# Dimitrinov74/Domain-Specific-Image-Compression

Hardware: AMD Instinct MI355X
Metric: 256x256 satellite patches encoded/s per GPU; bpp + MS-SSIM vs reference (higher is better)
Workload: dtype f32 (Winograd contractions as split-bf16 MFMA with fp32 accumulate); 1 GPU; batch=64/GPU 256x256x3 synthetic patches, modelv2 encode->decode (g_a,h_a,round,h_s,Student-t/Gaussian rate,g_s) + bpp + MS-SSIM[.3,.5,.2] on GPU + CDF tables and range coder (z,y strings) on GPU [BASELINE config 3]; global_batch=64, parallelism=per-image sharding x1, one all-reduce of 4 fp64, weights=synthetic seed 1 (checkpoints absent from the reference)

## Files before the change

### domain-specific-image-compression_amd/csrc/dsic_math.h

```cpp
#pragma once
#include <stdint.h>

#if defined(__HIPCC__)
#define DM_HD __host__ __device__ inline
#else
#define DM_HD inline
#endif

namespace dsic {
namespace dm {

#define DM_LN2_HI 6.93147180369123816490e-01
#define DM_LN2_LO 1.90821492927058770002e-10
#define DM_INV_LN2 1.44269504088896338700e+00
#define DM_SQRT2 1.41421356237309514547e+00
#define DM_INV_SQRT_PI 5.64189583547756279280e-01
#define DM_HALF_LOG_2PI 9.18938533204672780563e-01

DM_HD double from_bits(uint64_t b) {
  union {
    uint64_t u;
    double d;
  } v;
  v.u = b;
// ... 120 lines not shown
  for (int m = 1; m <= 400; ++m) {
    const double dm_ = (double)m, m2 = 2.0 * dm_;
    double aa = dm_ * (b - dm_) * x / ((qam + m2) * (a + m2));
    d = 1.0 + aa * d;
    if (d < TINY && d > -TINY) d = TINY;
    c = 1.0 + aa / c;
    if (c < TINY && c > -TINY) c = TINY;
    d = 1.0 / d;
    h = h * d * c;
    aa = -(a + dm_) * (qab + dm_) * x / ((a + m2) * (qap + m2));
    d = 1.0 + aa * d;
    if (d < TINY && d > -TINY) d = TINY;
    c = 1.0 + aa / c;
    if (c < TINY && c > -TINY) c = TINY;
    d = 1.0 / d;
    const double del = d * c;
    h = h * del;
    double dev = del - 1.0;
    if (dev < 0) dev = -dev;
    if (dev < 3e-16) break;
  }
  return h;
}

DM_HD double betainc(double a, double b, double x, double xc) {
  if (x <= 0.0) return 0.0;
  if (xc <= 0.0) return 1.0;
  const double lbeta = lgamma(a + b) - lgamma(a) - lgamma(b);
  const double front = exp(lbeta + a * log(x) + b * log(xc));
  if (x < (a + 1.0) / (a + b + 2.0)) return front * betacf(a, b, x) / a;
  return 1.0 - front * betacf(b, a, xc) / b;
}

DM_HD double student_t_cdf(double t, double nu) {
  const double t2 = t * t;
  const double den = nu + t2;
  const double x = nu / den, xc = t2 / den;
  const double tail = 0.5 * betainc(0.5 * nu, 0.5, x, xc);
  return t > 0 ? 1.0 - tail : tail;
}


DM_HD double erf_pos(double u) {
  if (u < 1.5) {
    const double u2 = u * u;
    double term = u, sum = u;
    for (int n = 1; n < 200; ++n) {
      term = term * (2.0 * u2) / (double)(2 * n + 1);
      sum = sum + term;
      if (term < sum * 1e-17) break;
    }
    return 2.0 * DM_INV_SQRT_PI * exp(-u2) * sum;
  }
  if (u > 6.0) return 1.0;
  return 1.0 - erfc_pos(u);
}

DM_HD float erff_rn(float a) {
  const double u = (double)a;
  if (u != u) return a;
  return u < 0 ? -(float)erf_pos(-u) : (float)erf_pos(u);
}

DM_HD float gaussian_cdf_f32(float x) {
  const float a = x / 1.41421354f;
  const float e = erff_rn(a);
  const float s = 1.0f + e;
  return 0.5f * s;
}

DM_HD float sum_f32_torch(const float* p, int n) {
// ... 57 lines not shown
```

### domain-specific-image-compression_amd/csrc/entropy.hip

```cpp
#include "common.h"
#include "dsic_math.h"

namespace dsic {

__global__ __launch_bounds__(256) void support_kernel(const float* __restrict__ y,
                                                      const float* __restrict__ z,
                                                      int* __restrict__ meta, int64_t ny, int64_t nz,
                                                      int tail) {
  __shared__ float red[2][4];
  __shared__ int bad_any;
  const int b = blockIdx.x;
  for (int which = 0; which < 2; ++which) {
    const float* p = which ? z + (size_t)b * nz : y + (size_t)b * ny;
    const int64_t n = which ? nz : ny;
    float mn = p[0], mx = p[0];
    bool bad = false;
    for (int64_t i = threadIdx.x; i < n; i += 256) {
      const float v = p[i];
      bad |= !(fabsf(v) < 1.0e9f);
      mn = fminf(mn, v);
      mx = fmaxf(mx, v);
    }
#pragma unroll
    for (int o = 32; o > 0; o >>= 1) {
      mn = fminf(mn, __shfl_down(mn, o, 64));
      mx = fmaxf(mx, __shfl_down(mx, o, 64));
    }
    if (threadIdx.x == 0) bad_any = 0;
    __syncthreads();
    if ((threadIdx.x & 63) == 0) {
      red[0][threadIdx.x >> 6] = mn;
      red[1][threadIdx.x >> 6] = mx;
    }
    if (__any(bad) && (threadIdx.x & 63) == 0) atomicOr(&bad_any, 1);
// ... 42 lines not shown
  __builtin_amdgcn_wave_barrier();
  for (int k = lane; k < L; k += 64) {
    uint32_t u16 = 0;
    if (k > 0) {
      float sc = F[k - 1] * 65535.0f;
      if (sc < 0.0f) sc = 0.0f;
      if (sc > 65535.0f) sc = 65535.0f;
      u16 = (uint32_t)sc;
    }
    out[k] = (uint16_t)((u16 * (uint32_t)(65536 - L)) / 65535u + (uint32_t)k);
  }
}

template <bool STUDENT>
__global__ __launch_bounds__(256) void tables_kernel(const float* __restrict__ sigma,
                                                     const float* __restrict__ nu, int sb,
                                                     const int* __restrict__ meta, int meta_off,
                                                     uint16_t* __restrict__ tables, int C, int Lmax,
                                                     int ntables, int* __restrict__ err) {
  extern __shared__ float shm[];
  const int wave = threadIdx.x >> 6, lane = threadIdx.x & 63;
  const int tid = blockIdx.x * 4 + wave;
  if (tid >= ntables) return;
  const int b = tid / C, c = tid % C;
  const int smin = meta[4 * b + meta_off], L = meta[4 * b + meta_off + 1];
  if (L > Lmax || L < 1) {
    if (lane == 0) atomicOr(err, 1);
    return;
  }
  float* F = shm + (size_t)wave * (2 * Lmax + 1);
  float* pmf = F + Lmax + 1;
  const float sg = sigma[(size_t)b * sb + c];
  const float nv = STUDENT ? nu[(size_t)b * sb + c] : 0.0f;
  for (int k = lane; k <= L; k += 64)
    F[k] = STUDENT ? dm::table_cdf_student(smin, k, sg, nv) : dm::table_cdf_gauss(smin, k, sg);
  __builtin_amdgcn_s_waitcnt(0xc07f);
  __builtin_amdgcn_wave_barrier();
  finish_table_wave(F, L, tables + ((size_t)b * C + c) * Lmax, pmf, lane);
}

__device__ __forceinline__ void put_bits(uint32_t* out32, int64_t cap_bits, int64_t off, uint32_t v,
                                         int len, int* overflow) {
  if (off + len > cap_bits) {
    *overflow = 1;
    return;
  }
  const int64_t w = off >> 5;
  const int s = (int)(off & 31), space = 32 - s;
  if (len <= space) {
    atomicOr(out32 + w, __builtin_bswap32(v << (space - len)));
  } else {
    const int rest = len - space;
    atomicOr(out32 + w, __builtin_bswap32(v >> rest));
    atomicOr(out32 + w + 1, __builtin_bswap32(v << (32 - rest)));
  }
}

__device__ __forceinline__ void put_ones(uint32_t* out32, int64_t cap_bits, int64_t off, uint32_t count,
                                         int* overflow) {
  while (count > 0) {
    const int len = count > 32 ? 32 : (int)count;
    put_bits(out32, cap_bits, off, len == 32 ? 0xFFFFFFFFu : ((1u << len) - 1u), len, overflow);
    off += len;
    count -= len;
  }
}

#ifndef ENC_SELECT
#define ENC_SELECT 1
#endif
template <int J>
__device__ __forceinline__ void wlane(uint32_t& rec, uint32_t v) {
  asm volatile("v_writelane_b32 %0, %1, %2" : "+v"(rec) : "s"(v), "n"(J));
}

template <int J>
__device__ __forceinline__ uint32_t rlane(uint32_t v) {
  uint32_t r;
  asm volatile("v_readlane_b32 %0, %1, %2" : "=s"(r) : "v"(v), "n"(J));
  return r;
}

template <int J>
__device__ __forceinline__ void enc_step(uint32_t& low, uint32_t& lowm1, uint32_t& span, uint32_t& cl,
                                         uint32_t& ch, uint32_t clo16, uint32_t chi16, uint32_t& rec_low,
                                         uint32_t& rec_high) {
  const uint32_t cl_next = J < 63 ? rlane<(J < 63 ? J + 1 : 63)>(clo16) : 0u;
  const uint32_t ch_next = J < 63 ? rlane<(J < 63 ? J + 1 : 63)>(chi16) : 0u;
  uint32_t lo_add, hi_add;
#if ENC_SELECT
  {
    const uint32_t ml = __umulhi(span, cl), mh = __umulhi(span, ch);
    lo_add = span ? ml : cl;
    hi_add = span ? mh : ch;
  }
// ... 168 lines not shown
        if (pendv == 0) {
          put_bits(dst32, cap_bits, off, bitsv, (int)nbv, &overflow);
        } else {
          const uint32_t first = bitsv >> (nbv - 1);
          put_bits(dst32, cap_bits, off, first, 1, &overflow);
          if (!first) put_ones(dst32, cap_bits, off + 1, pendv, &overflow);
          else if (off + 1 + (int64_t)pendv > cap_bits) overflow = 1;
          if (nbv > 1)
            put_bits(dst32, cap_bits, off + 1 + pendv, bitsv & ((1u << (nbv - 1)) - 1u), (int)nbv - 1, &overflow);
        }
      }
      base_bits += (int64_t)__builtin_amdgcn_readlane((int)incl, 63);
    }
    cur = nxt;
    sym1 = sym2;
  }
  pending += 1;
  const uint32_t bit = low < 0x40000000u ? 0u : 1u;
  if (lane == 0) {
    put_bits(dst32, cap_bits, base_bits, bit, 1, &overflow);
    if (!bit) put_ones(dst32, cap_bits, base_bits + 1, pending, &overflow);
    else if (base_bits + 1 + (int64_t)pending > cap_bits) overflow = 1;
  }
  const int64_t total_bits = base_bits + 1 + (int64_t)pending;
  if (__any(overflow)) {
    if (lane == 0) atomicOr(err, 4);
  }
  if (lane == 0) lengths[2 * b + which] = (int)((total_bits + 7) >> 3);
}

struct SplitGeom {
  int B, M, HWy, N, HWz, Lmax, per_element_y;
  int64_t ny, nz;
  __device__ __forceinline__ void stream(int s, int& which, int& b, int64_t& n, int64_t& base) const {
    which = s < B ? 1 : 0;
    b = which ? s : s - B;
    n = which ? ny : nz;
    base = which ? (int64_t)b * ny : (int64_t)B * ny + (int64_t)b * nz;
  }
};

__global__ __launch_bounds__(256) void enc_pack_kernel(const float* __restrict__ y, const float* __restrict__ z,
                                                       const int* __restrict__ meta, const uint16_t* __restrict__ tab_y,
                                                       const uint16_t* __restrict__ tab_z, SplitGeom G,
                                                       uint32_t* __restrict__ pairs, int* __restrict__ err) {
  int which, b;
  int64_t n, base;
  G.stream(blockIdx.y, which, b, n, base);
  const int HW = which ? G.HWy : G.HWz, Lmax = G.Lmax;
  const bool per_element = which && G.per_element_y;
  const float* sym = which ? y + (size_t)b * n : z + (size_t)b * n;
  const uint16_t* tab = (which ? tab_y + (size_t)b * (per_element ? (size_t)G.M * G.HWy : (size_t)G.M) * Lmax
                               : tab_z + (size_t)b * G.N * Lmax);
  const int smin = meta[4 * b + (which ? 0 : 2)], L = meta[4 * b + (which ? 1 : 3)];
  if (L > Lmax || L < 1) return;
  for (int64_t g = (int64_t)blockIdx.x * 256 + threadIdx.x; g < n; g += (int64_t)gridDim.x * 256) {
    const int c = (int)(g / HW);
    int sc = (int)sym[g] - smin;
    if (sc < 0 || sc >= L) {
      atomicOr(err, 2);
      sc = 0;
    }
    const uint16_t* t = tab + (size_t)(per_element ? g : (int64_t)c) * Lmax;
    const uint32_t c_low = t[sc];
    const uint32_t c_high = (sc == L - 1) ? 0x10000u : (uint32_t)t[sc + 1];
    pairs[base + g] = c_low | ((c_high - 1u) << 16);
  }
}

template <int J>
__device__ __forceinline__ void chain_step(uint32_t& low, uint32_t& lowm1, uint32_t& span, uint32_t& cl, uint32_t& ch,
                                           uint32_t pv, uint32_t& rec_low, uint32_t& rec_high) {
  const uint32_t pn = J < 63 ? rlane<(J < 63 ? J + 1 : 63)>(pv) : 0u;
// ... 61 lines not shown
    chain_steps8<40>(low, lowm1, span, cl, ch, cur, rl, rh);
    chain_steps8<48>(low, lowm1, span, cl, ch, cur, rl, rh);
    chain_steps8<56>(low, lowm1, span, cl, ch, cur, rl, rh);
    __builtin_amdgcn_raw_buffer_store_b32(rl, rlo, voff, g * 4u, 0);
    __builtin_amdgcn_raw_buffer_store_b32(rh, rhi, voff, g * 4u, 0);
    cur = n1;
    n1 = n2;
  }
  const int cnt = (int)((uint32_t)n - g);
  if (cnt > 0) {
    uint32_t rl = 0, rh = 0;
    for (int j = 0; j < cnt; ++j) {
      const uint32_t pr = __builtin_amdgcn_readlane(cur, j);
      const uint32_t cl = pr << 16, ch = (pr & 0xFFFF0000u) + 0x10000u;
      const uint32_t lo_add = span ? __umulhi(span, cl) : cl;
      const uint32_t hi_add = ch ? (span ? __umulhi(span, ch) : ch) : span;
      const uint32_t low1 = low + lo_add, high1 = lowm1 + hi_add, span1 = hi_add - lo_add;
      asm volatile("s_mov_b32 m0, %4\n\ts_nop 3\n\tv_writelane_b32 %0, %2, m0\n\tv_writelane_b32 %1, %3, m0"
                   : "+v"(rl), "+v"(rh)
                   : "s"(low1), "s"(high1), "s"(j));
      const int nb = __builtin_clz(low1 ^ high1);
      const int m = __builtin_clz(((high1 | ~low1) << 1) << nb);
      const int sh = nb + m;
      span = span1 << sh;
      low = (low1 << sh) & 0x7FFFFFFFu;
      lowm1 = low - 1u;
    }
    __builtin_amdgcn_raw_buffer_store_b32(rl, rlo, voff, g * 4u, 0);
    __builtin_amdgcn_raw_buffer_store_b32(rh, rhi, voff, g * 4u, 0);
  }
  if (threadIdx.x == 0) final_low[s] = low;
}

constexpr int PLACE_THREADS = 1024;

__global__ __launch_bounds__(PLACE_THREADS) void enc_place_kernel(const int* __restrict__ meta, SplitGeom G,
                                                                  const uint32_t* __restrict__ rec_low,
                                                                  const uint32_t* __restrict__ rec_high,
                                                                  const uint32_t* __restrict__ final_low,
                                                                  uint8_t* __restrict__ out, int64_t cap_y,
                                                                  int64_t cap_z, int* __restrict__ lengths,
                                                                  int* __restrict__ err) {
  __shared__ uint32_t sc_a[PLACE_THREADS], sc_t[PLACE_THREADS];
  __shared__ uint64_t sc_l[PLACE_THREADS];
  const int s = blockIdx.x, tid = threadIdx.x;
  int which, b;
  int64_t n, base;
  G.stream(s, which, b, n, base);
  const int L = meta[4 * b + (which ? 1 : 3)];
  if (L > G.Lmax || L < 1) {
    if (tid == 0) {
      atomicOr(err, 1);
      lengths[2 * b + which] = 0;
    }
    return;
  }
  const int64_t stride = cap_z + cap_y;
  uint32_t* dst32 = (uint32_t*)(out + (size_t)b * stride + (which ? cap_z : 0));
  const int64_t cap_bits = (which ? cap_y : cap_z) * 8;
  const uint32_t* rlo = rec_low + base;
  const uint32_t* rhi = rec_high + base;
  const int64_t per = (n + PLACE_THREADS - 1) / PLACE_THREADS;
  const int64_t j0 = (int64_t)tid * per < n ? (int64_t)tid * per : n;
  const int64_t j1 = j0 + per < n ? j0 + per : n;

  uint32_t t = 0, head = 0;
  uint64_t len = 0;
  for (int64_t j = j0; j < j1; ++j) {
    const uint32_t lo = rlo[j], hi = rhi[j];
    const uint32_t nb = (uint32_t)__builtin_clz(lo ^ hi);
    const uint32_t m = (uint32_t)__builtin_clz((((hi | ~lo) << nb) << 1) | 1u);
    if (nb) {
      len += nb + t;
      head = 1;
      t = 0;
    }
    t += m;
  }
  sc_a[tid] = head ? 0u : 1u;
  sc_t[tid] = t;
  __syncthreads();
  for (int o = 1; o < PLACE_THREADS; o <<= 1) {
    uint32_t pa = 1, pt = 0;
    if (tid >= o) {
      pa = sc_a[tid - o];
      pt = sc_t[tid - o];
    }
    __syncthreads();
    if (tid >= o) {
      const uint32_t a = sc_a[tid];
      sc_t[tid] = (a ? pt : 0u) + sc_t[tid];
      sc_a[tid] = pa & a;
    }
    __syncthreads();
  }
  const uint32_t carry_in = tid ? sc_t[tid - 1] : 0u;
  const uint32_t pend_final = sc_t[PLACE_THREADS - 1];
  const uint64_t mylen = len + (head ? (uint64_t)carry_in : 0u);
  __syncthreads();
  sc_l[tid] = mylen;
  __syncthreads();
  for (int o = 1; o < PLACE_THREADS; o <<= 1) {
    const uint64_t v = tid >= o ? sc_l[tid - o] : 0u;
    __syncthreads();
    sc_l[tid] += v;
    __syncthreads();
  }
  const int64_t total = (int64_t)sc_l[PLACE_THREADS - 1];
  int64_t off = (int64_t)(sc_l[tid] - mylen);

  int overflow = 0;
  uint32_t pend = carry_in;
  for (int64_t j = j0; j < j1; ++j) {
    const uint32_t lo = rlo[j], hi = rhi[j];
    const uint32_t nbv = (uint32_t)__builtin_clz(lo ^ hi);
    const uint32_t m = (uint32_t)__builtin_clz((((hi | ~lo) << nbv) << 1) | 1u);
    if (nbv) {
      const uint32_t bitsv = lo >> (32u - nbv);
      const uint32_t pendv = pend;
      if (pendv == 0) {
        put_bits(dst32, cap_bits, off, bitsv, (int)nbv, &overflow);
      } else {
        const uint32_t first = bitsv >> (nbv - 1);
        put_bits(dst32, cap_bits, off, first, 1, &overflow);
        if (!first) put_ones(dst32, cap_bits, off + 1, pendv, &overflow);
        else if (off + 1 + (int64_t)pendv > cap_bits) overflow = 1;
        if (nbv > 1)
          put_bits(dst32, cap_bits, off + 1 + pendv, bitsv & ((1u << (nbv - 1)) - 1u), (int)nbv - 1, &overflow);
      }
      off += nbv + pendv;
      pend = 0;
    }
    pend += m;
  }
  if (tid == 0) {
    const uint32_t pending = pend_final + 1u;
    const uint32_t bit = final_low[s] < 0x40000000u ? 0u : 1u;
    put_bits(dst32, cap_bits, total, bit, 1, &overflow);
    if (!bit) put_ones(dst32, cap_bits, total + 1, pending, &overflow);
    else if (total + 1 + (int64_t)pending > cap_bits) overflow = 1;
    lengths[2 * b + which] = (int)((total + 1 + (int64_t)pending + 7) >> 3);
  }
  if (overflow) atomicOr(err, 4);
}

__global__ __launch_bounds__(256) void range_decode_kernel(const uint8_t* __restrict__ in,
                                                           int64_t stride,
                                                           const int* __restrict__ lengths, int lstride,
                                                           int loff, const int* __restrict__ meta,
                                                           int meta_off,
                                                           const uint16_t* __restrict__ tables, int Lmax,
                                                           int C, int HW, float* __restrict__ out,
                                                           int* __restrict__ err, int B,
                                                           int per_element) {
  const int lane = threadIdx.x & 63;
  const int b = __builtin_amdgcn_readfirstlane(blockIdx.x * (blockDim.x >> 6) + (threadIdx.x >> 6));
  if (b >= B) return;
  const int smin = meta[4 * b + meta_off], L = meta[4 * b + meta_off + 1];
  if (L > Lmax || L < 1) {
    if (lane == 0) atomicOr(err, 1);
    return;
  }
  const uint16_t* gt = tables + (size_t)b * (per_element ? (size_t)C * HW : (size_t)C) * Lmax;
  const uint32_t* src32 = (const uint32_t*)(in + (size_t)b * stride);
  const int nbytes = lengths[b * lstride + loff];
  const int ndw = (nbytes + 3) >> 2;
  const int64_t n = (int64_t)C * HW;
  float* dst = out + (size_t)b * n;

  auto load_window = [&](int w0) -> uint32_t {
    const int k = w0 + lane;
    uint32_t v = 0;
    if (k < ndw) {
      v = __builtin_bswap32(src32[k]);
      const int valid = nbytes - 4 * k;
      if (valid < 4) v &= 0xFFFFFFFFu << (8 * (4 - valid));
// ... 131 lines not shown
          c_high = 0x10000u;
        }
      }
      ck0 = ck0_next;
      if (new_row) {
        row += 1;
        in_row = 0;
      } else {
        in_row += 1;
      }
      const int sidx = cnt - 1;
      if (lane == 0) dst[g] = (float)(sidx + smin);
      const uint32_t hi_add = (uint32_t)(((uint64_t)r * c_high + c_high) >> 16);
      const uint32_t lo_add = (uint32_t)(((uint64_t)r * c_low + c_low) >> 16);
      high = (low - 1u) + hi_add;
      low = low + lo_add;
      const int nb = __builtin_clz(low ^ high);
      low <<= nb;
      high = (high << nb) | ((1u << nb) - 1u);
      value = nb ? ((value << nb) | take(nb)) : value;
      const uint32_t e3 = (low << 1) & ~(high << 1);
      const int m = __builtin_clz(~e3);
      low = (low << m) & 0x7FFFFFFFu;
      high = (high << m) | 0x80000000u | ((1u << m) - 1u);
      value = m ? (((value << m) | take(m)) ^ 0x80000000u) : value;
    }
  }
}

}

using namespace dsic;

extern "C" int dsic_latent_support(const float* y_nchw, const float* z_nchw, int* meta, int B,
                                   int64_t n_y, int64_t n_z, int tail, void* stream) {
  DSIC_REQUIRE(y_nchw && z_nchw && meta, "latent_support: null pointer");
  DSIC_REQUIRE(B > 0 && n_y > 0 && n_z > 0 && tail >= 0, "latent_support: bad argument");
  hipLaunchKernelGGL(support_kernel, dim3(B), dim3(256), 0, (hipStream_t)stream, y_nchw, z_nchw, meta,
                     n_y, n_z, tail);
  return check_launch("latent_support");
}

static int tables_launch(bool student, const float* sigma, const float* nu, int per_image,
                         const int* meta, int meta_off, uint16_t* tables, int B, int C, int Lmax,
                         int* err, hipStream_t st) {
  DSIC_REQUIRE(sigma && meta && tables && err && (!student || nu), "cdf_tables: null pointer");
  DSIC_REQUIRE(B > 0 && C > 0 && Lmax >= 1 && Lmax <= 1000, "cdf_tables: Lmax=%d must be in [1,1000]", Lmax);
  const int ntables = B * C;
  const size_t shm = (size_t)4 * (2 * Lmax + 1) * sizeof(float);
  const int sb = per_image ? C : 0;
  if (student)
    hipLaunchKernelGGL(tables_kernel<true>, dim3(ceil_div(ntables, 4)), dim3(256), shm, st, sigma, nu, sb,
                       meta, meta_off, tables, C, Lmax, ntables, err);
  else
    hipLaunchKernelGGL(tables_kernel<false>, dim3(ceil_div(ntables, 4)), dim3(256), shm, st, sigma, nu, sb,
                       meta, meta_off, tables, C, Lmax, ntables, err);
  return check_launch("cdf_tables");
}

extern "C" int dsic_cdf_tables_gauss(const float* sigma_z, const int* meta, uint16_t* tables, int B,
                                     int N, int Lmax, int* err, void* stream) {
  return tables_launch(false, sigma_z, nullptr, 0, meta, 2, tables, B, N, Lmax, err, (hipStream_t)stream);
}

extern "C" int dsic_cdf_tables_student(const float* sigma, const float* nu, const int* meta,
                                       uint16_t* tables, int B, int rows, int Lmax, int* err,
                                       void* stream) {
  return tables_launch(true, sigma, nu, 1, meta, 0, tables, B, rows, Lmax, err, (hipStream_t)stream);
}

extern "C" int dsic_range_encode(const float* y_nchw, const float* z_nchw, const int* meta,
                                 const uint16_t* tab_y, const uint16_t* tab_z, int Lmax, int B, int M,
                                 int HWy, int N, int HWz, uint8_t* out, int64_t cap_y, int64_t cap_z,
                                 int* lengths, int* err, int streams_per_wg, int per_element_y,
                                 void* stream) {
  DSIC_REQUIRE(y_nchw && z_nchw && meta && tab_y && tab_z && out && lengths && err,
               "range_encode: null pointer");
  DSIC_REQUIRE(B > 0 && M > 0 && N > 0 && HWy > 0 && HWz > 0, "range_encode: empty latent");
  DSIC_REQUIRE(cap_y % 4 == 0 && cap_z % 4 == 0 && cap_y >= 8 && cap_z >= 8,
               "range_encode: capacities must be multiples of 4 and >= 8");
  DSIC_REQUIRE(streams_per_wg >= 1 && streams_per_wg <= 16, "range_encode: streams_per_wg must be in [1,16]");
  hipLaunchKernelGGL(range_encode_kernel, dim3(ceil_div(2 * B, streams_per_wg)), dim3(64 * streams_per_wg), 0,
                     (hipStream_t)stream,
                     y_nchw, z_nchw, meta, tab_y, tab_z, Lmax, M, HWy, N, HWz, out, cap_y, cap_z, lengths,
                     err, 2 * B, per_element_y ? 1 : 0);
  return check_launch("range_encode");
}

extern "C" int64_t dsic_range_encode_workspace_size(int B, int M, int HWy, int N, int HWz) {
  if (B <= 0 || M <= 0 || HWy <= 0 || N <= 0 || HWz <= 0) return -1;
  const int64_t total = (int64_t)B * ((int64_t)M * HWy + (int64_t)N * HWz);
  return 12 * total + 8 * (int64_t)B;
}

extern "C" int dsic_range_encode_ws(const float* y_nchw, const float* z_nchw, const int* meta,
                                    const uint16_t* tab_y, const uint16_t* tab_z, int Lmax, int B, int M,
                                    int HWy, int N, int HWz, uint8_t* out, int64_t cap_y, int64_t cap_z,
                                    int* lengths, int* err, int per_element_y, void* workspace,
                                    int64_t workspace_bytes, void* stream) {
  DSIC_REQUIRE(y_nchw && z_nchw && meta && tab_y && tab_z && out && lengths && err && workspace,
               "range_encode_ws: null pointer");
  DSIC_REQUIRE(B > 0 && M > 0 && N > 0 && HWy > 0 && HWz > 0, "range_encode_ws: empty latent");
  DSIC_REQUIRE(cap_y % 4 == 0 && cap_z % 4 == 0 && cap_y >= 8 && cap_z >= 8,
               "range_encode_ws: capacities must be multiples of 4 and >= 8");
  DSIC_REQUIRE(workspace_bytes >= dsic_range_encode_workspace_size(B, M, HWy, N, HWz),
               "range_encode_ws: workspace too small");
  SplitGeom G;
  G.B = B; G.M = M; G.HWy = HWy; G.N = N; G.HWz = HWz; G.Lmax = Lmax; G.per_element_y = per_element_y ? 1 : 0;
  G.ny = (int64_t)M * HWy;
  G.nz = (int64_t)N * HWz;
  DSIC_REQUIRE(G.ny < ((int64_t)1 << 29) && G.nz < ((int64_t)1 << 29), "range_encode_ws: string too long");
  const int64_t total = (int64_t)B * (G.ny + G.nz);
  uint32_t* pairs = (uint32_t*)workspace;
  uint32_t* rec_low = pairs + total;
  uint32_t* rec_high = rec_low + total;
  uint32_t* final_low = rec_high + total;
  hipStream_t st = (hipStream_t)stream;
  const int64_t nmax = G.ny > G.nz ? G.ny : G.nz;
  const int gx = (int)((nmax + 255) / 256 < 256 ? (nmax + 255) / 256 : 256);
  hipLaunchKernelGGL(enc_pack_kernel, dim3(gx, 2 * B), dim3(256), 0, st, y_nchw, z_nchw, meta, tab_y, tab_z, G, pairs,
                     err);
  int rc = check_launch("range_encode_ws: pack");
  if (rc != DSIC_OK) return rc;
  hipLaunchKernelGGL(enc_chain_kernel, dim3(2 * B), dim3(64), 0, st, pairs, meta, G, rec_low, rec_high, final_low);
  rc = check_launch("range_encode_ws: chain");
  if (rc != DSIC_OK) return rc;
  hipLaunchKernelGGL(enc_place_kernel, dim3(2 * B), dim3(PLACE_THREADS), 0, st, meta, G, rec_low, rec_high,
                     final_low, out, cap_y, cap_z, lengths, err);
  return check_launch("range_encode_ws: place");
}

extern "C" int dsic_range_decode(const uint8_t* in, int64_t stride, const int* lengths, int lstride,
                                 int loff, const int* meta, int meta_off, const uint16_t* tables,
                                 int Lmax, int B, int C, int HW, int per_element, float* out_nchw,
                                 int* err, void* stream) {
  DSIC_REQUIRE(in && lengths && meta && tables && out_nchw && err, "range_decode: null pointer");
  DSIC_REQUIRE(B > 0 && C > 0 && HW > 0 && Lmax >= 1, "range_decode: bad argument");
  DSIC_REQUIRE(meta_off == 0 || meta_off == 2, "range_decode: meta_off must be 0 (y) or 2 (z)");
  DSIC_REQUIRE(stride % 4 == 0, "range_decode: stride must be a multiple of 4");
  hipLaunchKernelGGL(range_decode_kernel, dim3(B), dim3(64), 0, (hipStream_t)stream, in, stride,
                     lengths, lstride, loff, meta, meta_off, tables, Lmax, C, HW, out_nchw, err, B, per_element ? 1 : 0);
  return check_launch("range_decode");
}

extern "C" int dsic_stream_create_masked(const uint32_t* mask_host, int words, void** stream_out) {
  DSIC_REQUIRE(mask_host && stream_out && words >= 1, "stream_create_masked: bad argument");
  hipStream_t st = nullptr;
  hipError_t e = hipExtStreamCreateWithCUMask(&st, (uint32_t)words, mask_host);
  if (e != hipSuccess) {
    set_error("hipExtStreamCreateWithCUMask: %s", hipGetErrorString(e));
    return DSIC_EHIP;
  }
  *stream_out = (void*)st;
  return DSIC_OK;
}
extern "C" int dsic_stream_destroy(void* stream) {
  hipError_t e = hipStreamDestroy((hipStream_t)stream);
  if (e != hipSuccess) {
    set_error("hipStreamDestroy: %s", hipGetErrorString(e));
    return DSIC_EHIP;
  }
  return DSIC_OK;
// ... 33 lines not shown
```

### domain-specific-image-compression_amd/lib.py

```python
from __future__ import annotations

import ctypes
import os
from ctypes import c_int, c_int64, c_void_p

HERE = os.path.dirname(os.path.abspath(__file__))
LIB_PATH = os.path.join(HERE, "libdsic_hip.so")

DSIC_OK, DSIC_EINVAL, DSIC_EHIP = 0, 1, 2
ACT_NONE, ACT_GDN, ACT_IGDN, ACT_RELU = 0, 1, 2, 3

_P = c_void_p
SIGNATURES = {
    "dsic_last_error": (ctypes.c_char_p, []),
    "dsic_abi_version": (c_int, []),
    "dsic_split_bf16": (c_int, []),
    "dsic_set_split_bf16": (c_int, [c_int]),
    "dsic_packed_conv_weight_floats": (c_int64, [c_int, c_int, c_int]),
    "dsic_pack_conv_weight": (c_int, [_P, _P, c_int, c_int, c_int, _P]),
    "dsic_pack_convT_weight": (c_int, [_P, _P, c_int, c_int, _P]),
    "dsic_convT_image_weight_floats": (c_int64, [c_int]),
    "dsic_pack_convT_image_weight": (c_int, [_P, _P, c_int, c_int, _P]),
    "dsic_image_to_nhwc8": (c_int, [_P, _P, c_int, c_int, c_int, c_int, _P]),
    "dsic_nhwc_to_nchw": (c_int, [_P, _P, c_int, c_int, c_int, c_int, _P]),
    "dsic_nchw_to_nhwc": (c_int, [_P, _P, c_int, c_int, c_int, c_int, _P]),
    "dsic_reflect_pad_br": (c_int, [_P, _P, c_int, c_int, c_int, c_int, c_int, _P]),
    "dsic_normalize_bands": (c_int, [_P, _P, _P, c_int, c_int, _P]),
    "dsic_conv2d_nhwc": (c_int, [_P, _P, _P, _P, _P, _P, c_int, c_int, c_int, c_int, c_int,
                                 c_int, c_int, c_int, _P]),
    "dsic_wino_weight_floats": (c_int64, [c_int, c_int]),
    "dsic_pack_wino_weight": (c_int, [_P, _P, c_int, c_int, _P]),
    "dsic_conv3x3_wino_nhwc": (c_int, [_P, _P, _P, _P, _P, _P, c_int, c_int, c_int, c_int, c_int, c_int, c_int, c_int,
                                       _P, _P]),
    "dsic_pack_wino_s2_weight": (c_int, [_P, _P, c_int, c_int, _P]),
    "dsic_pack_wino_convT_weight": (c_int, [_P, _P, c_int, c_int, _P]),
    "dsic_conv_transpose2d_wino_nhwc": (c_int, [_P, _P, _P, _P, _P, _P, c_int, c_int, c_int, c_int, c_int, c_int, _P,
                                                _P]),
    "dsic_wino_bf16_planes": (c_int, []),
    "dsic_wino_bf16_weight_bytes": (c_int64, [c_int, c_int]),
    "dsic_split_wino_weight_bf16": (c_int, [_P, _P, c_int, c_int, c_int, _P]),
# ... 97 lines not shown
```

Measured before the change: 10900 images/s.

## Parallelize range-coder bit placement across wave slices and share Gaussian CDF rows

Splits the single 1024-thread-per-stream bit placement into two kernels: one that summarizes fixed slices of each string per wave (pending-count and bit length via wave scans), and one that prefix-combines those slice summaries and emits bits through a per-wave shared-memory window before flushing with atomics. This exposes many more waves than the old one-block-per-stream design and removes its block-wide barrier-heavy scans. The change also adds a Gaussian table kernel that computes one shared CDF row per channel and reuses it across 16 images, and makes the Student-t table computation exploit symmetry so each tail evaluation fills two entries. Along the way it adds an ablation macro that can skip stages, which is off by default, plus an environment override for the library path. The cost is extra workspace, two launches instead of one, and atomic ORs on global words at slice boundaries.

```diff
diff --git a/domain-specific-image-compression_amd/csrc/dsic_math.h b/domain-specific-image-compression_amd/csrc/dsic_math.h
--- a/domain-specific-image-compression_amd/csrc/dsic_math.h
+++ b/domain-specific-image-compression_amd/csrc/dsic_math.h
@@ -176,11 +176,15 @@
   return 1.0 - front * betacf(b, a, xc) / b;
 }
 
-DM_HD double student_t_cdf(double t, double nu) {
+DM_HD double student_t_tail(double t, double nu) {
   const double t2 = t * t;
   const double den = nu + t2;
   const double x = nu / den, xc = t2 / den;
-  const double tail = 0.5 * betainc(0.5 * nu, 0.5, x, xc);
+  return 0.5 * betainc(0.5 * nu, 0.5, x, xc);
+}
+
+DM_HD double student_t_cdf(double t, double nu) {
+  const double tail = student_t_tail(t, nu);
   return t > 0 ? 1.0 - tail : tail;
 }
 
diff --git a/domain-specific-image-compression_amd/csrc/entropy.hip b/domain-specific-image-compression_amd/csrc/entropy.hip
--- a/domain-specific-image-compression_amd/csrc/entropy.hip
+++ b/domain-specific-image-compression_amd/csrc/entropy.hip
@@ -1,5 +1,7 @@
 #include "common.h"
 #include "dsic_math.h"
+
+#include <climits>
 
 namespace dsic {
 
@@ -108,11 +110,75 @@
   float* pmf = F + Lmax + 1;
   const float sg = sigma[(size_t)b * sb + c];
   const float nv = STUDENT ? nu[(size_t)b * sb + c] : 0.0f;
-  for (int k = lane; k <= L; k += 64)
-    F[k] = STUDENT ? dm::table_cdf_student(smin, k, sg, nv) : dm::table_cdf_gauss(smin, k, sg);
+  if (STUDENT && smin <= 0 && smin + L >= 1) {
+    const int whi = smin + L > 1 - smin ? smin + L : 1 - smin;
+    for (int w = 1 + lane; w <= whi; w += 64) {
+      const double tail = dm::student_t_tail((double)((float)w - 0.5f) / (double)sg, (double)nv);
+      if (w <= smin + L) F[w - smin] = (float)(1.0 - tail);
+      if (1 - w >= smin) F[1 - w - smin] = (float)tail;
+    }
+  } else {
+    for (int k = lane; k <= L; k += 64)
+      F[k] = STUDENT ? dm::table_cdf_student(smin, k, sg, nv) : dm::table_cdf_gauss(smin, k, sg);
+  }
   __builtin_amdgcn_s_waitcnt(0xc07f);
   __builtin_amdgcn_wave_barrier();
   finish_table_wave(F, L, tables + ((size_t)b * C + c) * Lmax, pmf, lane);
+}
+
+constexpr int ZT_IMGS = 16;
+
+__global__ __launch_bounds__(256) void gauss_tables_kernel(const float* __restrict__ sigma,
+                                                           const int* __restrict__ meta,
+                                                           uint16_t* __restrict__ tables, int B, int C, int Lmax,
+                                                           int rowmax, int* __restrict__ err) {
+  extern __shared__ float shm[];
+  __shared__ int ulo, uhi;
+  const int wave = threadIdx.x >> 6, lane = threadIdx.x & 63;
+  const int c = blockIdx.x, b0 = blockIdx.y * ZT_IMGS;
+  const int b1 = B - b0 < ZT_IMGS ? B : b0 + ZT_IMGS;
+  const float sg = sigma[c];
+  if (wave == 0) {
+    int lo = INT_MAX, hi = INT_MIN;
+    if (b0 + lane < b1 && lane < ZT_IMGS) {
+      const int smin = meta[4 * (b0 + lane) + 2], L = meta[4 * (b0 + lane) + 3];
+      if (L >= 1 && L <= Lmax) {
+        lo = smin;
+        hi = smin + L;
+      }
+    }
+#pragma unroll
+    for (int o = 32; o > 0; o >>= 1) {
+      lo = min(lo, __shfl_xor(lo, o, 64));
+      hi = max(hi, __shfl_xor(hi, o, 64));
+    }
+    if (lane == 0) {
+      ulo = lo;
+      uhi = hi;
+    }
+  }
+  __syncthreads();
+  const int lo = ulo, hi = uhi;
+  const bool shared_row = hi >= lo && (int64_t)hi - lo < (int64_t)rowmax;
+  float* row = shm;
+  if (shared_row)
+    for (int u = lo + (int)threadIdx.x; u <= hi; u += 256) row[u - lo] = dm::table_cdf_gauss(u, 0, sg);
+  __syncthreads();
+  float* F = shm + rowmax + (size_t)wave * (2 * Lmax + 1);
+  float* pmf = F + Lmax + 1;
+  for (int b = b0 + wave; b < b1; b += 4) {
+    const int smin = meta[4 * b + 2], L = meta[4 * b + 3];
+    if (L > Lmax || L < 1) {
+      if (lane == 0) atomicOr(err, 1);
+      continue;
+    }
+    for (int k = lane; k <= L; k += 64) F[k] = shared_row ? row[smin + k - lo] : dm::table_cdf_gauss(smin, k, sg);
+    __builtin_amdgcn_s_waitcnt(0xc07f);
+    __builtin_amdgcn_wave_barrier();
+    finish_table_wave(F, L, tables + ((size_t)b * C + c) * Lmax, pmf, lane);
+    __builtin_amdgcn_s_waitcnt(0xc07f);
+    __builtin_amdgcn_wave_barrier();
+  }
 }
 
 __device__ __forceinline__ void put_bits(uint32_t* out32, int64_t cap_bits, int64_t off, uint32_t v,
@@ -137,6 +203,40 @@
   while (count > 0) {
     const int len = count > 32 ? 32 : (int)count;
     put_bits(out32, cap_bits, off, len == 32 ? 0xFFFFFFFFu : ((1u << len) - 1u), len, overflow);
+    off += len;
+    count -= len;
+  }
+}
+
+constexpr int PLACE_WIN = 512;
+__device__ __forceinline__ void or_word(uint32_t* out32, uint32_t* win, int64_t wbase, int64_t w, uint32_t v) {
+  const int64_t i = w - wbase;
+  if (i >= 0 && i < PLACE_WIN) atomicOr(win + i, v);
+  else atomicOr(out32 + w, v);
+}
+
+__device__ __forceinline__ void put_bits_w(uint32_t* out32, uint32_t* win, int64_t wbase, int64_t cap_bits,
+                                           int64_t off, uint32_t v, int len, int* overflow) {
+  if (off + len > cap_bits) {
+    *overflow = 1;
+    return;
+  }
+  const int64_t w = off >> 5;
+  const int s = (int)(off & 31), space = 32 - s;
+  if (len <= space) {
+    or_word(out32, win, wbase, w, __builtin_bswap32(v << (space - len)));
+  } else {
+    const int rest = len - space;
+    or_word(out32, win, wbase, w, __builtin_bswap32(v >> rest));
+    or_word(out32, win, wbase, w + 1, __builtin_bswap32(v << (32 - rest)));
+  }
+}
+
+__device__ __forceinline__ void put_ones_w(uint32_t* out32, uint32_t* win, int64_t wbase, int64_t cap_bits,
+                                           int64_t off, uint32_t count, int* overflow) {
+  while (count > 0) {
+    const int len = count > 32 ? 32 : (int)count;
+    put_bits_w(out32, win, wbase, cap_bits, off, len == 32 ? 0xFFFFFFFFu : ((1u << len) - 1u), len, overflow);
     off += len;
     count -= len;
   }
@@ -371,13 +471,31 @@
 struct SplitGeom {
   int B, M, HWy, N, HWz, Lmax, per_element_y;
   int64_t ny, nz;
+  int gy, gz;
+  int ky, kz;
   __device__ __forceinline__ void stream(int s, int& which, int& b, int64_t& n, int64_t& base) const {
     which = s < B ? 1 : 0;
     b = which ? s : s - B;
     n = which ? ny : nz;
     base = which ? (int64_t)b * ny : (int64_t)B * ny + (int64_t)b * nz;
   }
+  __device__ __forceinline__ void slice(int q, int& s, int& k, int& ks, int& gs, int& q0) const {
+    const int qz = q - B * ky;
+    const bool y = qz < 0;
+    ks = y ? ky : kz;
+    gs = y ? gy : gz;
+    s = y ? q / ky : B + qz / kz;
+    k = y ? q % ky : qz % kz;
+    q0 = q - k;
+  }
 };
+
+static inline void place_slicing(int64_t n, int& groups, int& slices) {
+  const int64_t ng = (n + 63) / 64;
+  const int64_t g = (ng + 255) / 256 > 8 ? (ng + 255) / 256 : 8;
+  groups = (int)g;
+  slices = (int)((ng + g - 1) / g);
+}
 
 __global__ __launch_bounds__(256) void enc_pack_kernel(const float* __restrict__ y, const float* __restrict__ z,
                                                        const int* __restrict__ meta, const uint16_t* __restrict__ tab_y,
@@ -505,116 +623,201 @@
   if (threadIdx.x == 0) final_low[s] = low;
 }
 
-constexpr int PLACE_THREADS = 1024;
-
-__global__ __launch_bounds__(PLACE_THREADS) void enc_place_kernel(const int* __restrict__ meta, SplitGeom G,
-                                                                  const uint32_t* __restrict__ rec_low,
-                                                                  const uint32_t* __restrict__ rec_high,
-                                                                  const uint32_t* __restrict__ final_low,
-                                                                  uint8_t* __restrict__ out, int64_t cap_y,
-                                                                  int64_t cap_z, int* __restrict__ lengths,
-                                                                  int* __restrict__ err) {
-  __shared__ uint32_t sc_a[PLACE_THREADS], sc_t[PLACE_THREADS];
-  __shared__ uint64_t sc_l[PLACE_THREADS];
-  const int s = blockIdx.x, tid = threadIdx.x;
+#ifndef PLACE_WAVES
+#define PLACE_WAVES 4
+#endif
+constexpr int PLACE_CHUNK = 8;
+
+__device__ __forceinline__ void place_load(const uint32_t* __restrict__ rlo, const uint32_t* __restrict__ rhi,
+                                           int64_t c0, int64_t j1, int lane, uint32_t (&lo)[PLACE_CHUNK],
+                                           uint32_t (&hi)[PLACE_CHUNK]) {
+#pragma unroll
+  for (int i = 0; i < PLACE_CHUNK; ++i) {
+    const int64_t j = c0 + i * 64 + lane;
+    lo[i] = j < j1 ? rlo[j] : 0u;
+    hi[i] = j < j1 ? rhi[j] : ~0u;
+  }
+}
+
+__device__ __forceinline__ void place_group(uint32_t lo, uint32_t hi, int lane, uint32_t& pending, uint32_t& nbv,
+                                            uint32_t& pendv) {
+  nbv = (uint32_t)__builtin_clz(lo ^ hi);
+  const uint32_t mv = (uint32_t)__builtin_clz((((hi | ~lo) << nbv) << 1) | 1u);
+  uint32_t T = mv;
+#pragma unroll
+  for (int o = 1; o < 64; o <<= 1) {
+    const uint32_t up = __shfl_up(T, o, 64);
+    if (lane >= o) T += up;
+  }
+  const uint32_t Tex = T - mv;
+  const uint64_t heads = __ballot(nbv > 0);
+  const uint64_t before = heads & ((1ull << lane) - 1ull);
+  const int hb = 63 - __builtin_clzll(before | 1ull);
+  const uint32_t Tex_h = __shfl(Tex, hb, 64);
+  const uint32_t pend_in = before ? Tex - Tex_h : pending + Tex;
+  pendv = nbv ? pend_in : 0u;
+  const int hl = 63 - __builtin_clzll(heads | 1ull);
+  const uint32_t T63 = __builtin_amdgcn_readlane(T, 63);
+  const uint32_t Tex_hl = __builtin_amdgcn_readlane(Tex, hl);
+  pending = heads ? T63 - Tex_hl : pending + T63;
+}
+
+__global__ __launch_bounds__(64 * PLACE_WAVES) void enc_place_sum_kernel(const int* __restrict__ meta, SplitGeom G,
+                                                                         const uint32_t* __restrict__ rec_low,
+                                                                         const uint32_t* __restrict__ rec_high,
+                                                                         uint2* __restrict__ slices) {
+  const int lane = threadIdx.x & 63;
+  const int q = __builtin_amdgcn_readfirstlane(blockIdx.x * PLACE_WAVES + (threadIdx.x >> 6));
+  if (q >= G.B * (G.ky + G.kz)) return;
+  int s, k, ks, gs, q0;
+  G.slice(q, s, k, ks, gs, q0);
+  int which, b;
+  int64_t n, base;
+  G.stream(s, which, b, n, base);
+  const int L = meta[4 * b + (which ? 1 : 3)];
+  if (L > G.Lmax || L < 1) return;
+  const uint32_t* rlo = rec_low + base;
+  const uint32_t* rhi = rec_high + base;
+  const int64_t j0 = (int64_t)k * gs * 64;
+  const int64_t j1 = j0 + (int64_t)gs * 64 < n ? j0 + (int64_t)gs * 64 : n;
+  uint32_t pending = 0, bits = 0, head = 0;
+  for (int64_t c0 = j0; c0 < j1; c0 += PLACE_CHUNK * 64) {
+    uint32_t lo[PLACE_CHUNK], hi[PLACE_CHUNK];
+    place_load(rlo, rhi, c0, j1, lane, lo, hi);
+#pragma unroll
+    for (int i = 0; i < PLACE_CHUNK; ++i) {
+      if (c0 + i * 64 >= j1) break;
+      uint32_t nbv, pendv;
+      place_group(lo[i], hi[i], lane, pending, nbv, pendv);
+      head |= __ballot(nbv > 0) ? 1u : 0u;
+      uint32_t len = nbv + pendv;
+#pragma unroll
+      for (int o = 32; o > 0; o >>= 1) len += __shfl_xor(len, o, 64);
+      bits += len;
+    }
+  }
+  if (lane == 0) slices[q] = make_uint2(pending, bits | (head << 31));
+}
+
+__global__ __launch_bounds__(64 * PLACE_WAVES) void enc_place_emit_kernel(
+    const int* __restrict__ meta, SplitGeom G, const uint32_t* __restrict__ rec_low,
+    const uint32_t* __restrict__ rec_high, const uint2* __restrict__ slices, const uint32_t* __restrict__ final_low,
+    uint8_t* __restrict__ out, int64_t cap_y, int64_t cap_z, int* __restrict__ lengths, int* __restrict__ err) {
+  const int lane = threadIdx.x & 63;
+  const int q = __builtin_amdgcn_readfirstlane(blockIdx.x * PLACE_WAVES + (threadIdx.x >> 6));
+  if (q >= G.B * (G.ky + G.kz)) return;
+  int s, k, ks, gs, q0;
+  G.slice(q, s, k, ks, gs, q0);
   int which, b;
   int64_t n, base;
   G.stream(s, which, b, n, base);
   const int L = meta[4 * b + (which ? 1 : 3)];
   if (L > G.Lmax || L < 1) {
-    if (tid == 0) {
+    if (k == 0 && lane == 0) {
       atomicOr(err, 1);
       lengths[2 * b + which] = 0;
     }
     return;
   }
+  const uint32_t* rlo = rec_low + base;
+  const uint32_t* rhi = rec_high + base;
+  const int64_t j0 = (int64_t)k * gs * 64;
+  const int64_t j1 = j0 + (int64_t)gs * 64 < n ? j0 + (int64_t)gs * 64 : n;
+  uint32_t lo[PLACE_CHUNK], hi[PLACE_CHUNK];
+  place_load(rlo, rhi, j0, j1, lane, lo, hi);
+  uint32_t pending = 0;
+  uint64_t off = 0;
+  for (int i0 = 0; i0 < k; i0 += 64) {
+    const int i = i0 + lane;
+    uint32_t a = 1u, t = 0u, len = 0u;
+    if (i < k) {
+      const uint2 r = slices[q0 + i];
+      t = r.x;
+      len = r.y & 0x7FFFFFFFu;
+      a = (r.y >> 31) ? 0u : 1u;
+    }
+    uint32_t A = a, Tm = t;
+#pragma unroll
+    for (int o = 1; o < 64; o <<= 1) {
+      const uint32_t pa = __shfl_up(A, o, 64), pt = __shfl_up(Tm, o, 64);
+      if (lane >= o) {
+        Tm = (A ? pt : 0u) + Tm;
+        A = pa & A;
+      }
+    }
+    uint32_t Ae = __shfl_up(A, 1, 64), Te = __shfl_up(Tm, 1, 64);
+    if (lane == 0) {
+      Ae = 1u;
+      Te = 0u;
+    }
+    const uint32_t cin = (Ae ? pending : 0u) + Te;
+    uint64_t bits = (uint64_t)len + (a ? 0u : cin);
+#pragma unroll
+    for (int o = 32; o > 0; o >>= 1) bits += __shfl_xor(bits, o, 64);
+    off += bits;
+    const uint32_t A63 = __builtin_amdgcn_readlane(A, 63), T63 = __builtin_amdgcn_readlane(Tm, 63);
+    pending = (A63 ? pending : 0u) + T63;
+  }
+
   const int64_t stride = cap_z + cap_y;
   uint32_t* dst32 = (uint32_t*)(out + (size_t)b * stride + (which ? cap_z : 0));
   const int64_t cap_bits = (which ? cap_y : cap_z) * 8;
-  const uint32_t* rlo = rec_low + base;
-  const uint32_t* rhi = rec_high + base;
-  const int64_t per = (n + PLACE_THREADS - 1) / PLACE_THREADS;
-  const int64_t j0 = (int64_t)tid * per < n ? (int64_t)tid * per : n;
-  const int64_t j1 = j0 + per < n ? j0 + per : n;
-
-  uint32_t t = 0, head = 0;
-  uint64_t len = 0;
-  for (int64_t j = j0; j < j1; ++j) {
-    const uint32_t lo = rlo[j], hi = rhi[j];
-    const uint32_t nb = (uint32_t)__builtin_clz(lo ^ hi);
-    const uint32_t m = (uint32_t)__builtin_clz((((hi | ~lo) << nb) << 1) | 1u);
-    if (nb) {
-      len += nb + t;
-      head = 1;
-      t = 0;
-    }
-    t += m;
-  }
-  sc_a[tid] = head ? 0u : 1u;
-  sc_t[tid] = t;
-  __syncthreads();
-  for (int o = 1; o < PLACE_THREADS; o <<= 1) {
-    uint32_t pa = 1, pt = 0;
-    if (tid >= o) {
-      pa = sc_a[tid - o];
-      pt = sc_t[tid - o];
-    }
-    __syncthreads();
-    if (tid >= o) {
-      const uint32_t a = sc_a[tid];
-      sc_t[tid] = (a ? pt : 0u) + sc_t[tid];
-      sc_a[tid] = pa & a;
-    }
-    __syncthreads();
-  }
-  const uint32_t carry_in = tid ? sc_t[tid - 1] : 0u;
-  const uint32_t pend_final = sc_t[PLACE_THREADS - 1];
-  const uint64_t mylen = len + (head ? (uint64_t)carry_in : 0u);
-  __syncthreads();
-  sc_l[tid] = mylen;
-  __syncthreads();
-  for (int o = 1; o < PLACE_THREADS; o <<= 1) {
-    const uint64_t v = tid >= o ? sc_l[tid - o] : 0u;
-    __syncthreads();
-    sc_l[tid] += v;
-    __syncthreads();
-  }
-  const int64_t total = (int64_t)sc_l[PLACE_THREADS - 1];
-  int64_t off = (int64_t)(sc_l[tid] - mylen);
-
   int overflow = 0;
-  uint32_t pend = carry_in;
-  for (int64_t j = j0; j < j1; ++j) {
-    const uint32_t lo = rlo[j], hi = rhi[j];
-    const uint32_t nbv = (uint32_t)__builtin_clz(lo ^ hi);
-    const uint32_t m = (uint32_t)__builtin_clz((((hi | ~lo) << nbv) << 1) | 1u);
-    if (nbv) {
-      const uint32_t bitsv = lo >> (32u - nbv);
-      const uint32_t pendv = pend;
-      if (pendv == 0) {
-        put_bits(dst32, cap_bits, off, bitsv, (int)nbv, &overflow);
-      } else {
-        const uint32_t first = bitsv >> (nbv - 1);
-        put_bits(dst32, cap_bits, off, first, 1, &overflow);
-        if (!first) put_ones(dst32, cap_bits, off + 1, pendv, &overflow);
-        else if (off + 1 + (int64_t)pendv > cap_bits) overflow = 1;
-        if (nbv > 1)
-          put_bits(dst32, cap_bits, off + 1 + pendv, bitsv & ((1u << (nbv - 1)) - 1u), (int)nbv - 1, &overflow);
-      }
-      off += nbv + pendv;
-      pend = 0;
-    }
-    pend += m;
-  }
-  if (tid == 0) {
-    const uint32_t pending = pend_final + 1u;
+  __shared__ uint32_t win_all[PLACE_WAVES][PLACE_WIN];
+  uint32_t* win = win_all[threadIdx.x >> 6];
+#pragma unroll
+  for (int i = lane; i < PLACE_WIN; i += 64) win[i] = 0u;
+  const int64_t wbase = (int64_t)(off >> 5);
+  for (int64_t c0 = j0; c0 < j1; c0 += PLACE_CHUNK * 64) {
+    if (c0 != j0) place_load(rlo, rhi, c0, j1, lane, lo, hi);
+#pragma unroll
+    for (int i = 0; i < PLACE_CHUNK; ++i) {
+      if (c0 + i * 64 >= j1) break;
+      uint32_t nbv, pendv;
+      place_group(lo[i], hi[i], lane, pending, nbv, pendv);
+      const uint32_t len = nbv + pendv;
+      uint32_t incl = len;
+#pragma unroll
+      for (int o = 1; o < 64; o <<= 1) {
+        const uint32_t up = __shfl_up(incl, o, 64);
+        if (lane >= o) incl += up;
+      }
+      const int64_t o = (int64_t)off + (int64_t)(incl - len);
+      if (nbv > 0) {
+        const uint32_t bitsv = lo[i] >> (32u - nbv);
+        if (pendv == 0) {
+          put_bits_w(dst32, win, wbase, cap_bits, o, bitsv, (int)nbv, &overflow);
+        } else {
+          const uint32_t first = bitsv >> (nbv - 1);
+          put_bits_w(dst32, win, wbase, cap_bits, o, first, 1, &overflow);
+          if (!first) put_ones_w(dst32, win, wbase, cap_bits, o + 1, pendv, &overflow);
+          else if (o + 1 + (int64_t)pendv > cap_bits) overflow = 1;
+          if (nbv > 1)
+            put_bits_w(dst32, win, wbase, cap_bits, o + 1 + pendv, bitsv & ((1u << (nbv - 1)) - 1u), (int)nbv - 1,
+                       &overflow);
+        }
+      }
+      off += (uint32_t)__builtin_amdgcn_readlane((int)incl, 63);
+    }
+  }
+  const int64_t wend = (int64_t)((off + 31) >> 5) - wbase;
+  const int nw = wend < PLACE_WIN ? (int)wend : PLACE_WIN;
+  __builtin_amdgcn_s_waitcnt(0xc07f);
+  __builtin_amdgcn_wave_barrier();
+  for (int i = lane; i < nw; i += 64) {
+    const uint32_t v = win[i];
+    if (v) atomicOr(dst32 + wbase + i, v);
+  }
+  if (k == ks - 1 && lane == 0) {
+    const int64_t total = (int64_t)off;
+    const uint32_t pend = pending + 1u;
     const uint32_t bit = final_low[s] < 0x40000000u ? 0u : 1u;
     put_bits(dst32, cap_bits, total, bit, 1, &overflow);
-    if (!bit) put_ones(dst32, cap_bits, total + 1, pending, &overflow);
-    else if (total + 1 + (int64_t)pending > cap_bits) overflow = 1;
-    lengths[2 * b + which] = (int)((total + 1 + (int64_t)pending + 7) >> 3);
-  }
-  if (overflow) atomicOr(err, 4);
+    if (!bit) put_ones(dst32, cap_bits, total + 1, pend, &overflow);
+    else if (total + 1 + (int64_t)pend > cap_bits) overflow = 1;
+    lengths[2 * b + which] = (int)((total + 1 + (int64_t)pend + 7) >> 3);
+  }
+  if (__any(overflow) && lane == 0) atomicOr(err, 4);
 }
 
 __global__ __launch_bounds__(256) void range_decode_kernel(const uint8_t* __restrict__ in,
@@ -812,10 +1015,25 @@
 
 using namespace dsic;
 
+#ifndef ENC_ABL
+#define ENC_ABL 0
+#endif
+#if ENC_ABL
+__device__ int enc_abl_err_sink;
+static int* abl_err(int* err) {
+  void* p = nullptr;
+  return hipGetSymbolAddress(&p, HIP_SYMBOL(enc_abl_err_sink)) == hipSuccess ? (int*)p : err;
+}
+#else
+static int* abl_err(int* err) { return err; }
+#endif
+
+
 extern "C" int dsic_latent_support(const float* y_nchw, const float* z_nchw, int* meta, int B,
                                    int64_t n_y, int64_t n_z, int tail, void* stream) {
   DSIC_REQUIRE(y_nchw && z_nchw && meta, "latent_support: null pointer");
   DSIC_REQUIRE(B > 0 && n_y > 0 && n_z > 0 && tail >= 0, "latent_support: bad argument");
+  if (ENC_ABL & 1) return DSIC_OK;
   hipLaunchKernelGGL(support_kernel, dim3(B), dim3(256), 0, (hipStream_t)stream, y_nchw, z_nchw, meta,
                      n_y, n_z, tail);
   return check_launch("latent_support");
@@ -826,15 +1044,22 @@
                          int* err, hipStream_t st) {
   DSIC_REQUIRE(sigma && meta && tables && err && (!student || nu), "cdf_tables: null pointer");
   DSIC_REQUIRE(B > 0 && C > 0 && Lmax >= 1 && Lmax <= 1000, "cdf_tables: Lmax=%d must be in [1,1000]", Lmax);
+  if (ENC_ABL & 2) return DSIC_OK;
+  err = abl_err(err);
   const int ntables = B * C;
   const size_t shm = (size_t)4 * (2 * Lmax + 1) * sizeof(float);
   const int sb = per_image ? C : 0;
-  if (student)
+  if (student) {
     hipLaunchKernelGGL(tables_kernel<true>, dim3(ceil_div(ntables, 4)), dim3(256), shm, st, sigma, nu, sb,
                        meta, meta_off, tables, C, Lmax, ntables, err);
-  else
+  } else if (sb == 0) {
+    const int rowmax = 4 * Lmax;
+    hipLaunchKernelGGL(gauss_tables_kernel, dim3(C, ceil_div(B, ZT_IMGS)), dim3(256), shm + rowmax * sizeof(float),
+                       st, sigma, meta, tables, B, C, Lmax, rowmax, err);
+  } else {
     hipLaunchKernelGGL(tables_kernel<false>, dim3(ceil_div(ntables, 4)), dim3(256), shm, st, sigma, nu, sb,
                        meta, meta_off, tables, C, Lmax, ntables, err);
+  }
   return check_launch("cdf_tables");
 }
 
@@ -867,10 +1092,18 @@
   return check_launch("range_encode");
 }
 
+static int64_t place_records(int B, int64_t ny, int64_t nz) {
+  int gy, ky, gz, kz;
+  place_slicing(ny, gy, ky);
+  place_slicing(nz, gz, kz);
+  return (int64_t)B * (ky + kz);
+}
+
 extern "C" int64_t dsic_range_encode_workspace_size(int B, int M, int HWy, int N, int HWz) {
   if (B <= 0 || M <= 0 || HWy <= 0 || N <= 0 || HWz <= 0) return -1;
-  const int64_t total = (int64_t)B * ((int64_t)M * HWy + (int64_t)N * HWz);
-  return 12 * total + 8 * (int64_t)B;
+  const int64_t ny = (int64_t)M * HWy, nz = (int64_t)N * HWz;
+  const int64_t total = (int64_t)B * (ny + nz);
+  return 12 * total + 8 * (int64_t)B + 8 + 8 * place_records(B, ny, nz);
 }
 
 extern "C" int dsic_range_encode_ws(const float* y_nchw, const float* z_nchw, const int* meta,
@@ -885,29 +1118,48 @@
                "range_encode_ws: capacities must be multiples of 4 and >= 8");
   DSIC_REQUIRE(workspace_bytes >= dsic_range_encode_workspace_size(B, M, HWy, N, HWz),
                "range_encode_ws: workspace too small");
+  err = abl_err(err);
   SplitGeom G;
   G.B = B; G.M = M; G.HWy = HWy; G.N = N; G.HWz = HWz; G.Lmax = Lmax; G.per_element_y = per_element_y ? 1 : 0;
   G.ny = (int64_t)M * HWy;
   G.nz = (int64_t)N * HWz;
   DSIC_REQUIRE(G.ny < ((int64_t)1 << 29) && G.nz < ((int64_t)1 << 29), "range_encode_ws: string too long");
+  place_slicing(G.ny, G.gy, G.ky);
+  place_slicing(G.nz, G.gz, G.kz);
+  const int64_t nslices = (int64_t)B * (G.ky + G.kz);
+  DSIC_REQUIRE(nslices < ((int64_t)1 << 30), "range_encode_ws: too many strings");
   const int64_t total = (int64_t)B * (G.ny + G.nz);
   uint32_t* pairs = (uint32_t*)workspace;
   uint32_t* rec_low = pairs + total;
   uint32_t* rec_high = rec_low + total;
   uint32_t* final_low = rec_high + total;
+  uint2* slices = (uint2*)(((uintptr_t)(final_low + 2 * B) + 7) & ~(uintptr_t)7);
   hipStream_t st = (hipStream_t)stream;
-  const int64_t nmax = G.ny > G.nz ? G.ny : G.nz;
-  const int gx = (int)((nmax + 255) / 256 < 256 ? (nmax + 255) / 256 : 256);
-  hipLaunchKernelGGL(enc_pack_kernel, dim3(gx, 2 * B), dim3(256), 0, st, y_nchw, z_nchw, meta, tab_y, tab_z, G, pairs,
-                     err);
-  int rc = check_launch("range_encode_ws: pack");
-  if (rc != DSIC_OK) return rc;
-  hipLaunchKernelGGL(enc_chain_kernel, dim3(2 * B), dim3(64), 0, st, pairs, meta, G, rec_low, rec_high, final_low);
-  rc = check_launch("range_encode_ws: chain");
-  if (rc != DSIC_OK) return rc;
-  hipLaunchKernelGGL(enc_place_kernel, dim3(2 * B), dim3(PLACE_THREADS), 0, st, meta, G, rec_low, rec_high,
-                     final_low, out, cap_y, cap_z, lengths, err);
-  return check_launch("range_encode_ws: place");
+  int rc = DSIC_OK;
+  if (!(ENC_ABL & 4)) {
+    const int64_t nmax = G.ny > G.nz ? G.ny : G.nz;
+    const int gx = (int)((nmax + 255) / 256 < 256 ? (nmax + 255) / 256 : 256);
+    hipLaunchKernelGGL(enc_pack_kernel, dim3(gx, 2 * B), dim3(256), 0, st, y_nchw, z_nchw, meta, tab_y, tab_z, G,
+                       pairs, err);
+    rc = check_launch("range_encode_ws: pack");
+    if (rc != DSIC_OK) return rc;
+  }
+  if (!(ENC_ABL & 16)) {
+    hipLaunchKernelGGL(enc_chain_kernel, dim3(2 * B), dim3(64), 0, st, pairs, meta, G, rec_low, rec_high, final_low);
+    rc = check_launch("range_encode_ws: chain");
+    if (rc != DSIC_OK) return rc;
+  }
+  if (!(ENC_ABL & 8)) {
+    const int nwg = (int)((nslices + PLACE_WAVES - 1) / PLACE_WAVES);
+    hipLaunchKernelGGL(enc_place_sum_kernel, dim3(nwg), dim3(64 * PLACE_WAVES), 0, st, meta, G, rec_low, rec_high,
+                       slices);
+    rc = check_launch("range_encode_ws: place summarize");
+    if (rc != DSIC_OK) return rc;
+    hipLaunchKernelGGL(enc_place_emit_kernel, dim3(nwg), dim3(64 * PLACE_WAVES), 0, st, meta, G, rec_low, rec_high,
+                       slices, final_low, out, cap_y, cap_z, lengths, err);
+    rc = check_launch("range_encode_ws: place emit");
+  }
+  return rc;
 }
 
 extern "C" int dsic_range_decode(const uint8_t* in, int64_t stride, const int* lengths, int lstride,
diff --git a/domain-specific-image-compression_amd/lib.py b/domain-specific-image-compression_amd/lib.py
--- a/domain-specific-image-compression_amd/lib.py
+++ b/domain-specific-image-compression_amd/lib.py
@@ -5,7 +5,7 @@
 from ctypes import c_int, c_int64, c_void_p
 
 HERE = os.path.dirname(os.path.abspath(__file__))
-LIB_PATH = os.path.join(HERE, "libdsic_hip.so")
+LIB_PATH = os.environ.get("DSIC_LIB") or os.path.join(HERE, "libdsic_hip.so")
 
 DSIC_OK, DSIC_EINVAL, DSIC_EHIP = 0, 1, 2
 ACT_NONE, ACT_GDN, ACT_IGDN, ACT_RELU = 0, 1, 2, 3
```

New measurement: 11220 images/s, median of 6. 1.03x the previous value.
